# RustAudio/rodio

Measured on AMD Instinct MI355X. Metric: Msamples/s through resample+low_pass+mix pipeline, higher is better.
Workload: dtype f32; 1 GPU; 256 f32 stereo sources/GPU x 1048576 frames, 44.1->48 kHz linear resample + low_pass(200) + ordered Mixer sum, span_len=None; numpy default_rng(1234+s) U(-1,1)/256; in_frames=1048576, out_frames=1141308, channels=2, kernel=k_rlm_chunk

## Files before the change

### rodio_amd/csrc/rh_pipeline_chunk.hip

```cpp
#include "rh_pipeline_dev.h"

namespace {

struct ChunkArgs {
    const uint32_t *m_lo;
    unsigned long long *halo;
    const float *lookT;
    const float *powM;
    const float *uni;
};
constexpr uint32_t kChunkMultiMax = 7;
struct ChunkMulti {
    struct Entry {
        Params p;
        ChunkArgs q;
    };
    uint32_t n;
    uint32_t first[kChunkMultiMax + 1];
    float *sum_out;
    Entry e[kChunkMultiMax];
};
static_assert(sizeof(ChunkMulti) <= 4096, "the kernarg segment");
#if defined(RH_CHUNK_DIAG) && RH_CHUNK_DIAG == 3
#define RH_CPH(i) { const unsigned long long cph_now = __builtin_readcyclecounter(); if (lane == 0) atomicAdd(p.ticket + 8 + (i), (uint32_t)(cph_now - cph_last)); cph_last = cph_now; }
#define RH_CPH_DECL unsigned long long cph_last = __builtin_readcyclecounter();
#else
#define RH_CPH(i)
#define RH_CPH_DECL
#endif
template <int R, int C, int KV, typename ST = float>
__device__ __forceinline__ void rlm_chunk_tile(const Params &p, const ChunkArgs &q, const uint32_t block) {
    typedef Chan<C> CH;
    typedef typename CH::V V;
    constexpr bool PCM = sizeof(ST) == 2;
    constexpr int NS = 2, H = 4;
    constexpr uint32_t FB = CH::kFB;
    constexpr uint32_t kStage = KV * 1024, P = kStage / FB;
    constexpr int NSI = PCM ? 2 * NS : NS;
    constexpr uint32_t kIn = PCM ? kStage / 2 : kStage;
    constexpr int G = PCM ? KV / 2 : KV;
    static_assert(KV % 2 == 0 && NSI * kIn == NS * kStage, "the ring's bytes, cut for either sample type");
    constexpr uint32_t MB = NS * kStage + 64;
    __shared__ __attribute__((aligned(1024))) unsigned char smem[MB + kStage + 64];
    lds_u8 *const lds = (lds_u8 *)smem;
    const uint32_t lds0 = (uint32_t)(uintptr_t)lds;
    typedef __attribute__((address_space(4))) const uint64_t cu64;
    typedef __attribute__((address_space(4))) const float cf32;
    typedef __attribute__((address_space(4))) const uint32_t cu32;
    cu64 *const desc = (cu64 *)(uintptr_t)p.srcs;
    cf32 *const dgain = (cf32 *)(uintptr_t)p.srcs;
    const int lane = threadIdx.x;
    uint32_t tile = block;
    if (!p.direct) {
        const uint32_t x = block & 7u;
        const uint32_t k = __builtin_amdgcn_readfirstlane(lane == 0 ? atomicAdd(p.ticket + 32u * (1u + x), 1u) - p.shard_base : 0u);
        tile = x + 8u * k;
        if (tile >= p.n_tiles) return;
    }
#ifdef RH_CHUNK_RAGSIM
    const uint32_t Ns = p.eq_frames;
    const uint32_t S = 2u * tile < p.n_tiles ? p.n_sources : (uint32_t)(((uint64_t)p.n_sources * 2u * (p.n_tiles - tile)) / p.n_tiles);
#else
    const uint32_t Ns = p.eq_frames, S = p.n_sources;
#endif
    const uint32_t m_lo = ((cu32 *)(uintptr_t)q.m_lo)[tile], m_hi = ((cu32 *)(uintptr_t)q.m_lo)[tile + 1];
    const uint32_t m0 = m_lo + (uint32_t)lane * R;
    int nfl;
    uint32_t n_t_v;
    float pwv[4];
    {
        const uint32_t n_t = m_hi - m_lo;
        nfl = (int)n_t - lane * R < 0 ? 0 : ((int)n_t - lane * R > R ? R : (int)n_t - lane * R);
        const uint32_t nl0 = (n_t + R - 1) / R;
        const uint32_t v = nl0 ? n_t - (nl0 - 1) * R : 0;
        n_t_v = n_t;
        asm volatile("v_mov_b32 %0, %1" : "=v"(n_t_v) : "s"(n_t));
        const float *pw = q.powM + 4 * v;
#pragma unroll
        for (int k = 0; k < 4; ++k) {
            pwv[k] = pw[k];
            asm volatile("" : "+v"(pwv[k]));
        }
    }
    const bool first = (m0 == 0);

    const uint32_t nvec = PCM ? Ns * C / 8 : Ns * C / 4;
    const uint32_t v0 = tile * (G * 64);
    uint32_t goff[G];
#pragma unroll
    for (int k = 0; k < G; ++k) {
        uint32_t j = v0 + (uint32_t)k * 64 + lane;
        j = j < nvec ? j : nvec - 1;
        goff[k] = j * 16;
    }
    const bool lin = v0 + (uint32_t)(G * 64) <= nvec;
    auto stage_source = [&](uint32_t s_, uint32_t stage) {
        const void *data = (const void *)(uintptr_t)desc[4 * (uint64_t)s_];
        if (lin) {
            glds16_run<G>(data, goff[0], lds0 + stage * kIn);
        } else {
#pragma unroll
            for (int k = 0; k < G; ++k) glds16(data, goff[k], lds0 + stage * kIn + k * 1024);
        }
    };
    if (S) stage_source(0, 0);
    if (S > 1) stage_source(1, 1);
    if constexpr (PCM) {
        if (S > 2) stage_source(2, 2);
        if (S > 3) stage_source(3, 3);
    }
    const Tables *__restrict__ tb = p.tabs;
    float lM[4], b15[4], b31[4], kM[4];
    constexpr int NHV = H * FB / 16;
    const uint32_t Jc = p.J < tile ? p.J : tile;
    int want_look = (uint32_t)lane < Jc ? 1 : 0;
    uint64_t a_halo_pub = (uint64_t)(uintptr_t)(q.halo + (uint64_t)tile * 8 + (uint32_t)(lane >= 64 - NHV ? lane - (64 - NHV) : 0) * 4);
    uint64_t a_halo_poll = (uint64_t)(uintptr_t)(q.halo + (uint64_t)(tile ? tile - 1 : 0) * 8 + (lane < H * C ? lane : 0));
    uint64_t a_gran_pub = (uint64_t)(uintptr_t)(p.gran + (uint64_t)tile * 4 + (lane < 2 * C ? lane : 0));
    uint64_t a_gran_poll = (uint64_t)(uintptr_t)(p.gran + (uint64_t)(tile ? tile - 1 - (want_look ? lane : 0) : 0) * 4);
    uint64_t a_out = (uint64_t)(uintptr_t)(p.out + ((uint64_t)m_lo + (uint32_t)lane) * C);
    uint32_t epoch_v = p.epoch;
    float U = q.uni[lane < 61 ? lane : 60];
    asm volatile("" : "+v"(want_look), "+v"(a_halo_pub), "+v"(a_halo_poll), "+v"(a_gran_pub), "+v"(a_gran_poll), "+v"(a_out), "+v"(epoch_v), "+v"(U));
    {
        const uint32_t Jc0 = Jc;
        const float *kp = q.lookT + ((uint64_t)tile * p.J + ((uint32_t)lane < Jc0 ? lane : 0)) * 4;
#pragma unroll
        for (int k = 0; k < 4; ++k) {
            lM[k] = tb->laneM[lane][k];
            b15[k] = tb->bc15M[lane][k];
            b31[k] = tb->bc31M[lane][k];
            kM[k] = kp[k];
        }
    }
    int offA[R + 2];
    float wgt[R + 2];
    {
        const int64_t fbase = (int64_t)tile * P;
        Cursor c = cursor_at(first ? 0 : m0 - 2, p);
#pragma unroll
        for (int rr = 0; rr < R + 2; ++rr) {
#if defined(RH_CHUNK_DIAG) && RH_CHUNK_DIAG == 2
            offA[rr] = (int)MB + rr * 8;
            wgt[rr] = 0.5f;
            continue;
#endif
            const bool dummy = first && rr < 2;
            uint64_t i;
            uint32_t num;
            cursor_resolve(c, p, i, num);
            if (i + 1 >= Ns) {
                i = Ns - 1;
                num = 0;
            }
            int64_t f = (int64_t)i - fbase;
            f = f < -H ? -H : (f > (int64_t)P - 1 ? (int64_t)P - 1 : f);
            offA[rr] = dummy ? (int)MB : (int)MB + (int)f * (int)FB;
            wgt[rr] = dummy ? 0.0f : (float)num / p.Tf;
            if (!dummy) cursor_next(c, p);
        }
    }
    v4f acc[KV];
#pragma unroll
    for (int k = 0; k < KV; ++k) acc[k] = v4f{0.f, 0.f, 0.f, 0.f};
    if constexpr (!PCM) {
        uint32_t st = 0;
        float g_next = S ? dgain[4] : 0.f;
        for (uint32_t s_ = 0; s_ < S; ++s_) {
            const float g = g_next;
            g_next = s_ + 1 < S ? dgain[8 * (uint64_t)(s_ + 1) + 4] : 0.f;
            if (s_ + 1 < S) wait_vm<KV>();
            else wait_vm<0>();
            const lds_u8 *buf = lds + st * kStage;
            v4f v[KV];
#pragma unroll
            for (int k = 0; k < KV; ++k) v[k] = *(const lds_f4 *)(buf + k * 1024 + lane * 16);
            asm volatile("s_waitcnt lgkmcnt(0)" ::: "memory");
            if (s_ + 2 < S) stage_source(s_ + 2, st);
#pragma unroll
            for (int k = 0; k < KV; ++k) {
                acc[k].x = fma_(g, v[k].x, acc[k].x);
                acc[k].y = fma_(g, v[k].y, acc[k].y);
                acc[k].z = fma_(g, v[k].z, acc[k].z);
                acc[k].w = fma_(g, v[k].w, acc[k].w);
            }
            st ^= 1u;
        }
    } else {
        uint32_t st = 0;
        float g_next = S ? dgain[4] : 0.f;
        for (uint32_t s_ = 0; s_ < S; ++s_) {
            const float g = g_next;
            g_next = s_ + 1 < S ? dgain[8 * (uint64_t)(s_ + 1) + 4] : 0.f;
            const uint32_t left = S - 1 - s_;
            wait_groups<G, NSI>((int)(left < (uint32_t)(NSI - 1) ? left : (uint32_t)(NSI - 1)));
            const lds_u8 *buf = lds + st * kIn;
            v4i16 v[KV];
#pragma unroll
            for (int k = 0; k < KV; ++k) v[k] = *(const RH_LDS v4i16 *)(buf + k * 512 + lane * 8);
            asm volatile("s_waitcnt lgkmcnt(0)" ::: "memory");
            if (s_ + NSI < S) stage_source(s_ + NSI, st);
#pragma unroll
            for (int k = 0; k < KV; ++k) {
                acc[k].x = fma_(g, pcm16_f32(v[k].x), acc[k].x);
                acc[k].y = fma_(g, pcm16_f32(v[k].y), acc[k].y);
                acc[k].z = fma_(g, pcm16_f32(v[k].z), acc[k].z);
                acc[k].w = fma_(g, pcm16_f32(v[k].w), acc[k].w);
            }
            st = (st + 1u) & (uint32_t)(NSI - 1);
        }
    }
    RH_CPH_DECL
#if defined(RH_CHUNK_DIAG) && RH_CHUNK_DIAG < 3
    {
        float t = 0.f;
#pragma unroll
        for (int k = 0; k < KV; ++k) t += acc[k].x + acc[k].y + acc[k].z + acc[k].w;
#pragma unroll
        for (int rr = 0; rr < R + 2; ++rr) t += wgt[rr] + (float)offA[rr];
        p.out[(uint64_t)tile * 64 + lane] = t + lM[0] + b15[0] + b31[0] + kM[0] + (float)nfl + (first ? 1.f : 0.f);
        return;
    }
#endif
    if (lane >= 64 - NHV) {
        unsigned long long *hp = (unsigned long long *)(uintptr_t)a_halo_pub;
        const float e[4] = {acc[KV - 1].x, acc[KV - 1].y, acc[KV - 1].z, acc[KV - 1].w};
#pragma unroll
        for (int w = 0; w < 4; ++w) __hip_atomic_store(hp + w, ((unsigned long long)epoch_v << 32) | __float_as_uint(e[w]), __ATOMIC_RELAXED, __HIP_MEMORY_SCOPE_AGENT);
    }
#pragma unroll
    for (int k = 0; k < KV; ++k) *(lds_f4 *)(lds + MB + (uint32_t)(k * 64 + lane) * 16) = acc[k];
    if (lane == 0) *(lds_f4 *)(lds + MB + kStage) = v4f{0.f, 0.f, 0.f, 0.f};
    bool dead = false;
    if (tile == 0) {
        if (lane < H * C) *(RH_LDS float *)(lds + MB - H * FB + lane * 4) = 0.0f;
    } else {
        const bool want = lane < H * C;
        const unsigned long long *hp = (const unsigned long long *)(uintptr_t)a_halo_poll;
        unsigned long long hv = 0;
        bool ok = false;
        uint32_t spins = 0;
        while (true) {
            if (want && !ok) {
                hv = __hip_atomic_load(hp, __ATOMIC_RELAXED, __HIP_MEMORY_SCOPE_AGENT);
                ok = (uint32_t)(hv >> 32) == epoch_v;
            }
            if (__all(ok || !want)) break;
            if (++spins > kSpinLimit) {
                if (lane == 0) atomicOr(p.status, 1u);
                dead = true;
                break;
            }
            __builtin_amdgcn_s_sleep(1);
        }
        if (want) *(RH_LDS float *)(lds + MB - H * FB + lane * 4) = dead ? __builtin_nanf("") : __uint_as_float((uint32_t)hv);
    }
    asm volatile("s_waitcnt lgkmcnt(0)" ::: "memory");
    __builtin_amdgcn_wave_barrier();
    RH_CPH(0)

    const float b0 = readlane_f(U, 0), c1 = readlane_f(U, 1), c2 = readlane_f(U, 2), na1 = -readlane_f(U, 3), na2 = -readlane_f(U, 4);
    V out[R];
    V E1 = CH::zero(), E2 = CH::zero();
    {
        V ta[R + 2], tb2[R + 2];
#pragma unroll
        for (int rr = 0; rr < R + 2; ++rr) {
            ta[rr] = CH::ld_lds(lds + offA[rr]);
            tb2[rr] = CH::ld_lds(lds + offA[rr] + FB);
        }
        auto tap = [&](int rr) -> V {
            V x;
#pragma unroll
            for (int ch = 0; ch < C; ++ch) CH::set(x, ch, fma_(CH::get(tb2[rr], ch) - CH::get(ta[rr], ch), wgt[rr], CH::get(ta[rr], ch)));
            return x;
        };
        V x2 = first ? CH::zero() : tap(0);
        V x1 = first ? CH::zero() : tap(1);
        V w1 = CH::zero(), w2 = CH::zero();
#pragma unroll
        for (int r = 0; r < R; ++r) {
            const V x = tap(r + 2);
            V w;
#pragma unroll
            for (int ch = 0; ch < C; ++ch) {
                const float wc = fma_(na1, CH::get(w1, ch), fma_(na2, CH::get(w2, ch), fma_(c2, CH::get(x2, ch), c1 * CH::get(x1, ch))));
                CH::set(w, ch, wc);
                CH::set(out[r], ch, fma_(b0, CH::get(x, ch), wc));
            }
            w2 = w1;
            w1 = w;
            x2 = x1;
            x1 = x;
            E1 = vsel(r + 1 == nfl, w1, E1);
            E2 = vsel(r + 1 == nfl, w2, E2);
        }
    }
    RH_CPH(1)
    float Pq[2 * C];
#pragma unroll
    for (int k = 0; k < 2 * C; ++k) Pq[k] = 0.f;
    {
        const float Tm[4] = {readlane_f(U, 5), readlane_f(U, 6), readlane_f(U, 7), readlane_f(U, 8)};
#pragma unroll
        for (int ch = 0; ch < C; ++ch) mat_acc(Tm, CH::get(E1, ch), CH::get(E2, ch), Pq[2 * ch], Pq[2 * ch + 1]);
    }
    float own[2 * C];
#pragma unroll
    for (int k = 0; k < 2 * C; ++k) own[k] = Pq[k];
    scan_states(Pq, ScanStepsLanes{U}, b15, b31);
    {
        const uint32_t n_t = (uint32_t)__builtin_amdgcn_readfirstlane((int)n_t_v);
        float A[2 * C];
        tile_aggregate(own, Pq, pwv, (int)((n_t + R - 1) / R), A);
        if (lane < 2 * C) {
            float ev = A[0];
#pragma unroll
            for (int k = 1; k < 2 * C; ++k) ev = lane == k ? A[k] : ev;
            __hip_atomic_store((unsigned long long *)(uintptr_t)a_gran_pub, ((unsigned long long)epoch_v << 32) | __float_as_uint(ev), __ATOMIC_RELAXED, __HIP_MEMORY_SCOPE_AGENT);
        }
    }
    float Q[2 * C];
#pragma unroll
    for (int k = 0; k < 2 * C; ++k) Q[k] = dpp0<kDppWaveShr1, 0xf>(Pq[k]);
    RH_CPH(2)
    float c[2 * C];
#pragma unroll
    for (int k = 0; k < 2 * C; ++k) c[k] = 0.f;
    if (tile > 0) {
        const bool want = want_look != 0;
        const unsigned long long *gp = (const unsigned long long *)(uintptr_t)a_gran_poll;
        unsigned long long gv[2 * C];
#pragma unroll
        for (int k = 0; k < 2 * C; ++k) gv[k] = 0;
        bool ok = false;
        uint32_t spins = 0;
        while (true) {
            if (want && !ok) {
                bool all = true;
#pragma unroll
                for (int k = 0; k < 2 * C; ++k) {
                    gv[k] = __hip_atomic_load(gp + k, __ATOMIC_RELAXED, __HIP_MEMORY_SCOPE_AGENT);
                    all = all && ((uint32_t)(gv[k] >> 32) == epoch_v);
                }
                ok = all;
            }
            if (__all(ok || !want)) break;
            if (++spins > kSpinLimit) {
                if (lane == 0) atomicOr(p.status, 1u);
                dead = true;
                break;
            }
            __builtin_amdgcn_s_sleep(4);
        }
        if (lane == 0 && spins) atomicAdd(p.status + 1, spins);
        if (want && ok && !dead) {
#pragma unroll
            for (int ch = 0; ch < C; ++ch) mat_acc(kM, __uint_as_float((uint32_t)gv[2 * ch]), __uint_as_float((uint32_t)gv[2 * ch + 1]), c[2 * ch], c[2 * ch + 1]);
        }
#pragma unroll
        for (int k = 0; k < 2 * C; ++k) {
            c[k] += dpp0<kDppRowShr + 1, 0xf>(c[k]);
            c[k] += dpp0<kDppRowShr + 2, 0xf>(c[k]);
            c[k] += dpp0<kDppRowShr + 4, 0xf>(c[k]);
            c[k] += dpp0<kDppRowShr + 8, 0xf>(c[k]);
            c[k] = readlane_f(c[k], 15) + readlane_f(c[k], 31);
        }
    }
    if (dead) {
#pragma unroll
        for (int k = 0; k < 2 * C; ++k) c[k] = __builtin_nanf("");
    }
    RH_CPH(3)
#pragma unroll
    for (int ch = 0; ch < C; ++ch) mat_acc(lM, c[2 * ch], c[2 * ch + 1], Q[2 * ch], Q[2 * ch + 1]);
    tile_store<R, C>(lds, lane, [&] { return (uint32_t)__builtin_amdgcn_readfirstlane((int)n_t_v); }, [&] { return (float *)(uintptr_t)a_out; }, [&](int r) {
        V y;
#pragma unroll
        for (int ch = 0; ch < C; ++ch) CH::set(y, ch, fma_(readlane_f(U, 25 + 2 * r), Q[2 * ch], fma_(readlane_f(U, 26 + 2 * r), Q[2 * ch + 1], CH::get(out[r], ch))));
        return y;
    });
    RH_CPH(4)
}
template <int R, int C, int KV>
__global__ __launch_bounds__(64, 2) void k_rlm_chunk(const Params p, const ChunkArgs q) {
    rlm_chunk_tile<R, C, KV>(p, q, blockIdx.x);
}
template <int R, int C, int KV>
__global__ __launch_bounds__(64, 2) void k_rlm_chunk_pcm16(const Params p, const ChunkArgs q) {
    rlm_chunk_tile<R, C, KV, int16_t>(p, q, blockIdx.x);
}
template <int R, int C, int KV>
__global__ __launch_bounds__(64, 2) void k_rlm_chunk_multi(const ChunkMulti m) {
    uint32_t k = 0;
#pragma unroll
    for (uint32_t i = 1; i < kChunkMultiMax; ++i) k += (i < m.n && blockIdx.x >= m.first[i]) ? 1u : 0u;
    uint32_t b0 = 0;
#pragma unroll
    for (uint32_t i = 1; i < kChunkMultiMax; ++i) b0 = (i == k) ? m.first[i] : b0;
    k = __builtin_amdgcn_readfirstlane(k);
    typedef const __attribute__((address_space(4))) unsigned char *cbytes;
    cbytes e = (cbytes)__builtin_amdgcn_kernarg_segment_ptr() + offsetof(ChunkMulti, e) + (size_t)k * sizeof(ChunkMulti::Entry);
    Params p;
    ChunkArgs q;
    typedef const __attribute__((address_space(4))) uint32_t *cwords;
    static_assert(sizeof(Params) % 4 == 0 && sizeof(ChunkArgs) % 4 == 0 && offsetof(ChunkMulti::Entry, q) % 4 == 0, "copied word by word");
    {
        cwords wp = (cwords)(e + offsetof(ChunkMulti::Entry, p)), wq = (cwords)(e + offsetof(ChunkMulti::Entry, q));
        uint32_t *dp = reinterpret_cast<uint32_t *>(&p), *dq = reinterpret_cast<uint32_t *>(&q);
#pragma unroll
        for (uint32_t i = 0; i < sizeof(Params) / 4; ++i) dp[i] = wp[i];
#pragma unroll
        for (uint32_t i = 0; i < sizeof(ChunkArgs) / 4; ++i) dq[i] = wq[i];
    }
    rlm_chunk_tile<R, C, KV>(p, q, blockIdx.x - b0);
}

#if defined(RH_CLS_DIAG) && RH_CLS_DIAG == 9
__device__ unsigned long long g_cls_stamp[2048 * 8 * 8];
#define RH_CLS_STAMP(i) { if (lane == 0 && tile < 2048 && k < 8) g_cls_stamp[((uint64_t)tile * 8 + k) * 8 + (i)] = wall_clock64(); }
#else
#define RH_CLS_STAMP(i)
#endif
#define RH_PARG(T, e, f) (*(const __attribute__((address_space(4))) T *)((e) + offsetof(ChunkMulti::Entry, p) + offsetof(Params, f)))
#define RH_QARG(T, e, f) (*(const __attribute__((address_space(4))) T *)((e) + offsetof(ChunkMulti::Entry, q) + offsetof(ChunkArgs, f)))
template <int R, int C, int KV>
__global__ __launch_bounds__(128, 2) void k_rlm_chunk_classes(const ChunkMulti m) {
    typedef Chan<C> CH;
    typedef typename CH::V V;
    constexpr int NS = 2, H = 4;
    constexpr uint32_t FB = CH::kFB;
    constexpr uint32_t kStage = KV * 1024, P = kStage / FB;
    constexpr uint32_t kCtl = NS * kStage;
    constexpr uint32_t kImg = kStage + 128;
    constexpr uint32_t MB0 = kCtl + 64 + 64;
    __shared__ __attribute__((aligned(1024))) unsigned char smem[kCtl + 64 + 2 * kImg];
    lds_u8 *const lds = (lds_u8 *)smem;
    const uint32_t lds0 = (uint32_t)(uintptr_t)lds;
    typedef __attribute__((address_space(4))) const uint64_t cu64;
    typedef __attribute__((address_space(4))) const float cf32;
    typedef __attribute__((address_space(4))) const uint32_t cu32;
    typedef const __attribute__((address_space(4))) unsigned char *cbytes;
    const cbytes kseg = (cbytes)__builtin_amdgcn_kernarg_segment_ptr();
    const int wave = __builtin_amdgcn_readfirstlane((int)(threadIdx.x >> 6));
    const int lane = (int)(threadIdx.x & 63u);
    const uint32_t n_cls = m.n;
    const Params &p0 = m.e[0].p;
    const uint32_t tile = blockIdx.x;
    const uint32_t Ns = p0.eq_frames;
    auto entry = [&](uint32_t k) -> cbytes { return kseg + offsetof(ChunkMulti, e) + (size_t)k * sizeof(ChunkMulti::Entry); };
    auto ctl_read = [&](uint32_t which) -> uint32_t {
        uint32_t v;
        asm volatile("ds_read_b32 %0, %1\n\ts_waitcnt lgkmcnt(0)" : "=v"(v) : "v"(lds0 + kCtl + which * 4) : "memory");
        return (uint32_t)__builtin_amdgcn_readfirstlane((int)v);
    };
    auto ctl_write = [&](uint32_t which, uint32_t v) {
        asm volatile("s_waitcnt lgkmcnt(0)" ::: "memory");
        if (lane == 0) *(RH_LDS uint32_t *)(lds + kCtl + which * 4) = v;
        asm volatile("s_waitcnt lgkmcnt(0)" ::: "memory");
    };
    if (wave == 0) {
        if (lane < 2) *(RH_LDS uint32_t *)(lds + kCtl + lane * 4) = 0u;
    }
    asm volatile("s_waitcnt lgkmcnt(0)\n\ts_barrier" ::: "memory");
    if (wave == 0) {
        const uint32_t nvec = Ns * C / 4;
        const uint32_t v0 = tile * (KV * 64);
        uint32_t goff[KV];
#pragma unroll
        for (int k = 0; k < KV; ++k) {
            uint32_t j = v0 + (uint32_t)k * 64 + lane;
            j = j < nvec ? j : nvec - 1;
            goff[k] = j * 16;
        }
        const bool lin = v0 + (uint32_t)(KV * 64) <= nvec;
        auto stage_source = [&](cu64 *desc, uint32_t s_, uint32_t stage) {
            const void *data = (const void *)(uintptr_t)desc[4 * (uint64_t)s_];
            if (lin) {
                glds16_run<KV>(data, goff[0], lds0 + stage * kStage);
            } else {
#pragma unroll
                for (int k = 0; k < KV; ++k) glds16(data, goff[k], lds0 + stage * kStage + k * 1024);
            }
        };
        constexpr int NHV = H * FB / 16;
        __builtin_amdgcn_s_setprio(3);
        uint32_t kc = 0, sc = 0;
        cu64 *ndesc = (cu64 *)(uintptr_t)RH_PARG(uint64_t, entry(0), srcs);
        uint32_t nS = RH_PARG(uint32_t, entry(0), n_sources);
        uint32_t nstage = 0;
        auto request_next = [&]() {
            if (kc >= n_cls) return false;
            stage_source(ndesc, sc, nstage);
            nstage ^= 1u;
            if (++sc == nS) {
                sc = 0;
                if (++kc < n_cls) {
                    ndesc = (cu64 *)(uintptr_t)RH_PARG(uint64_t, entry(kc), srcs);
                    nS = RH_PARG(uint32_t, entry(kc), n_sources);
                }
            }
            return true;
        };
        uint32_t ahead = 0;
        if (request_next()) ++ahead;
        if (request_next()) ++ahead;
        uint32_t st = 0;
        for (uint32_t k = 0; k < n_cls; ++k) {
            const cbytes e = entry(k);
            cf32 *const dgain = (cf32 *)(uintptr_t)RH_PARG(uint64_t, e, srcs);
            const uint32_t S = RH_PARG(uint32_t, e, n_sources);
            v4f acc[KV];
#pragma unroll
            for (int i = 0; i < KV; ++i) acc[i] = v4f{0.f, 0.f, 0.f, 0.f};
            float g_next = S ? dgain[4] : 0.f;
            for (uint32_t s_ = 0; s_ < S; ++s_) {
                const float g = g_next;
                g_next = s_ + 1 < S ? dgain[8 * (uint64_t)(s_ + 1) + 4] : 0.f;
                if (ahead > 1) wait_vm<KV>();
                else wait_vm<0>();
                --ahead;
                const lds_u8 *buf = lds + st * kStage;
                v4f v[KV];
#pragma unroll
                for (int i = 0; i < KV; ++i) v[i] = *(const lds_f4 *)(buf + i * 1024 + lane * 16);
                asm volatile("s_waitcnt lgkmcnt(0)" ::: "memory");
                if (request_next()) ++ahead;
#pragma unroll
                for (int i = 0; i < KV; ++i) {
                    acc[i].x = fma_(g, v[i].x, acc[i].x);
                    acc[i].y = fma_(g, v[i].y, acc[i].y);
                    acc[i].z = fma_(g, v[i].z, acc[i].z);
                    acc[i].w = fma_(g, v[i].w, acc[i].w);
                }
                st ^= 1u;
            }
            RH_CLS_STAMP(0)
            if (lane >= 64 - NHV) {
                unsigned long long *hp = (unsigned long long *)(uintptr_t)RH_QARG(uint64_t, e, halo) + (uint64_t)tile * 8 + (uint32_t)(lane - (64 - NHV)) * 4;
                const uint32_t epoch = RH_PARG(uint32_t, e, epoch);
                const float ev[4] = {acc[KV - 1].x, acc[KV - 1].y, acc[KV - 1].z, acc[KV - 1].w};
#pragma unroll
                for (int w = 0; w < 4; ++w) __hip_atomic_store(hp + w, ((unsigned long long)epoch << 32) | __float_as_uint(ev[w]), __ATOMIC_RELAXED, __HIP_MEMORY_SCOPE_AGENT);
            }
            if (k >= 2) {
                uint32_t spins = 0;
                while (ctl_read(1) + 2 <= k) {
                    if (++spins > kSpinLimit) break;
                    __builtin_amdgcn_s_sleep(8);
                }
            }
            {
                lds_u8 *img = lds + MB0 + (k & 1u) * kImg;
#pragma unroll
                for (int i = 0; i < KV; ++i) *(lds_f4 *)(img + (uint32_t)(i * 64 + lane) * 16) = acc[i];
                if (lane == 0) *(lds_f4 *)(img + kStage) = v4f{0.f, 0.f, 0.f, 0.f};
            }
            ctl_write(0, k + 1);
            RH_CLS_STAMP(1)
        }
        return;
    }
    const ChunkArgs &q0 = m.e[0].q;
    const uint32_t m_lo = ((cu32 *)(uintptr_t)q0.m_lo)[tile], m_hi = ((cu32 *)(uintptr_t)q0.m_lo)[tile + 1];
    const uint32_t m0 = m_lo + (uint32_t)lane * R;
    const uint32_t n_t = m_hi - m_lo;
    const int nfl = (int)n_t - lane * R < 0 ? 0 : ((int)n_t - lane * R > R ? R : (int)n_t - lane * R);
    const uint32_t nl0 = (n_t + R - 1) / R;
    const uint32_t vlast = nl0 ? n_t - (nl0 - 1) * R : 0;
    const bool first = (m0 == 0);
    int offA[R + 2];
    float wgt[R + 2];
    {
        const int64_t fbase = (int64_t)tile * P;
        Cursor c = cursor_at(first ? 0 : m0 - 2, p0);
#pragma unroll
        for (int rr = 0; rr < R + 2; ++rr) {
            const bool dummy = first && rr < 2;
            uint64_t i;
            uint32_t num;
            cursor_resolve(c, p0, i, num);
            if (i + 1 >= Ns) {
                i = Ns - 1;
                num = 0;
            }
            int64_t f = (int64_t)i - fbase;
            f = f < -H ? -H : (f > (int64_t)P - 1 ? (int64_t)P - 1 : f);
            offA[rr] = dummy ? 0 : (int)f * (int)FB;
            wgt[rr] = dummy ? 0.0f : (float)num / p0.Tf;
            if (!dummy) cursor_next(c, p0);
        }
    }
    V ytot[R];
#pragma unroll
    for (int r = 0; r < R; ++r) ytot[r] = CH::zero();
    for (uint32_t k = 0; k < n_cls; ++k) {
        const cbytes e = entry(k);
        const Tables *__restrict__ tb = (const Tables *)(uintptr_t)RH_PARG(uint64_t, e, tabs);
        const uint32_t J = RH_PARG(uint32_t, e, J), epoch = RH_PARG(uint32_t, e, epoch);
        const uint32_t Jc = J < tile ? J : tile;
        const bool want_look = (uint32_t)lane < Jc;
        unsigned long long *const halo = (unsigned long long *)(uintptr_t)RH_QARG(uint64_t, e, halo);
        unsigned long long *const gran = (unsigned long long *)(uintptr_t)RH_PARG(uint64_t, e, gran);
        uint32_t *const status = (uint32_t *)(uintptr_t)RH_PARG(uint64_t, e, status);
        const float U = ((const float *)(uintptr_t)RH_QARG(uint64_t, e, uni))[lane < 61 ? lane : 60];
        float lM[4], b15[4], b31[4], kM[4], pwv[4];
        {
            const float *kp = (const float *)(uintptr_t)RH_QARG(uint64_t, e, lookT) + ((uint64_t)tile * J + (want_look ? lane : 0)) * 4;
            const float *pw = (const float *)(uintptr_t)RH_QARG(uint64_t, e, powM) + 4 * vlast;
#pragma unroll
            for (int i = 0; i < 4; ++i) {
                lM[i] = tb->laneM[lane][i];
                b15[i] = tb->bc15M[lane][i];
                b31[i] = tb->bc31M[lane][i];
                kM[i] = kp[i];
                pwv[i] = pw[i];
            }
        }
        lds_u8 *const img = lds + MB0 + (k & 1u) * kImg;
        {
            uint32_t spins = 0;
            while (ctl_read(0) <= k) {
                if (++spins > kSpinLimit) {
                    if (lane == 0) atomicOr(status, 1u);
                    break;
                }
                __builtin_amdgcn_s_sleep(8);
            }
        }
#if defined(RH_CLS_DIAG) && RH_CLS_DIAG == 1
        CH::set(ytot[0], 0, CH::get(ytot[0], 0) + lM[0] + b15[0] + b31[0] + kM[0] + pwv[0] + U + (float)offA[0] + wgt[1] + (float)nfl + (want_look ? 1.f : 0.f) + (float)(uintptr_t)halo + (float)(uintptr_t)gran + (float)(uintptr_t)status + (float)epoch);
        ctl_write(1, k + 1);
        continue;
#endif
        RH_CLS_STAMP(2)
        bool dead = false;
        if (tile == 0) {
            if (lane < H * C) *(RH_LDS float *)(img - H * FB + lane * 4) = 0.0f;
        } else {
            const bool want = lane < H * C;
            const unsigned long long *hp = halo + (uint64_t)(tile - 1) * 8 + (want ? lane : 0);
            unsigned long long hv = 0;
            bool ok = false;
            uint32_t spins = 0;
            while (true) {
                if (want && !ok) {
                    hv = __hip_atomic_load(hp, __ATOMIC_RELAXED, __HIP_MEMORY_SCOPE_AGENT);
                    ok = (uint32_t)(hv >> 32) == epoch;
                }
                if (__all(ok || !want)) break;
                if (++spins > kSpinLimit) {
                    if (lane == 0) atomicOr(status, 1u);
                    dead = true;
                    break;
                }
                __builtin_amdgcn_s_sleep(1);
            }
            if (want) *(RH_LDS float *)(img - H * FB + lane * 4) = dead ? __builtin_nanf("") : __uint_as_float((uint32_t)hv);
        }
        asm volatile("s_waitcnt lgkmcnt(0)" ::: "memory");
        __builtin_amdgcn_wave_barrier();
        RH_CLS_STAMP(3)
        const float b0 = readlane_f(U, 0), c1 = readlane_f(U, 1), c2 = readlane_f(U, 2), na1 = -readlane_f(U, 3), na2 = -readlane_f(U, 4);
        V out[R];
        V E1 = CH::zero(), E2 = CH::zero();
        {
            V ta[R + 2], tb2[R + 2];
#pragma unroll
            for (int rr = 0; rr < R + 2; ++rr) {
                ta[rr] = CH::ld_lds(img + offA[rr]);
                tb2[rr] = CH::ld_lds(img + offA[rr] + FB);
            }
            auto tap = [&](int rr) -> V {
                V x;
#pragma unroll
                for (int ch = 0; ch < C; ++ch) CH::set(x, ch, fma_(CH::get(tb2[rr], ch) - CH::get(ta[rr], ch), wgt[rr], CH::get(ta[rr], ch)));
                return x;
            };
            V x2 = first ? CH::zero() : tap(0);
            V x1 = first ? CH::zero() : tap(1);
            V w1 = CH::zero(), w2 = CH::zero();
#pragma unroll
            for (int r = 0; r < R; ++r) {
                const V x = tap(r + 2);
                V w;
#pragma unroll
                for (int ch = 0; ch < C; ++ch) {
                    const float wc = fma_(na1, CH::get(w1, ch), fma_(na2, CH::get(w2, ch), fma_(c2, CH::get(x2, ch), c1 * CH::get(x1, ch))));
                    CH::set(w, ch, wc);
                    CH::set(out[r], ch, fma_(b0, CH::get(x, ch), wc));
                }
                w2 = w1;
                w1 = w;
                x2 = x1;
                x1 = x;
                E1 = vsel(r + 1 == nfl, w1, E1);
                E2 = vsel(r + 1 == nfl, w2, E2);
            }
        }
        float Pq[2 * C];
#pragma unroll
        for (int i = 0; i < 2 * C; ++i) Pq[i] = 0.f;
        {
            const float Tm[4] = {readlane_f(U, 5), readlane_f(U, 6), readlane_f(U, 7), readlane_f(U, 8)};
#pragma unroll
            for (int ch = 0; ch < C; ++ch) mat_acc(Tm, CH::get(E1, ch), CH::get(E2, ch), Pq[2 * ch], Pq[2 * ch + 1]);
        }
        float own[2 * C];
#pragma unroll
        for (int i = 0; i < 2 * C; ++i) own[i] = Pq[i];
#define RH_CSCAN(K, N)                                                                             \
    {                                                                                              \
        float sq[2 * C];                                                                           \
        _Pragma("unroll") for (int i = 0; i < 2 * C; ++i) sq[i] = dpp0<kDppRowShr + N, 0xf>(Pq[i]); \
        const float sM[4] = {readlane_f(U, 9 + 4 * K), readlane_f(U, 10 + 4 * K), readlane_f(U, 11 + 4 * K), readlane_f(U, 12 + 4 * K)}; \
        _Pragma("unroll") for (int ch = 0; ch < C; ++ch) mat_acc(sM, sq[2 * ch], sq[2 * ch + 1], Pq[2 * ch], Pq[2 * ch + 1]); \
    }
        RH_CSCAN(0, 1)
        RH_CSCAN(1, 2)
        RH_CSCAN(2, 4)
        RH_CSCAN(3, 8)
#undef RH_CSCAN
        {
            float sq[2 * C];
#pragma unroll
            for (int i = 0; i < 2 * C; ++i) sq[i] = dpp0<kDppBcast15, 0xa>(Pq[i]);
#pragma unroll
            for (int ch = 0; ch < C; ++ch) mat_acc(b15, sq[2 * ch], sq[2 * ch + 1], Pq[2 * ch], Pq[2 * ch + 1]);
        }
        {
            float sq[2 * C];
#pragma unroll
            for (int i = 0; i < 2 * C; ++i) sq[i] = dpp0<kDppBcast31, 0xc>(Pq[i]);
#pragma unroll
            for (int ch = 0; ch < C; ++ch) mat_acc(b31, sq[2 * ch], sq[2 * ch + 1], Pq[2 * ch], Pq[2 * ch + 1]);
        }
        {
            const int nl = (int)nl0;
            float A[2 * C];
#pragma unroll
            for (int i = 0; i < 2 * C; ++i) A[i] = 0.f;
            if (nl >= 1) {
#pragma unroll
                for (int i = 0; i < 2 * C; ++i) A[i] = __int_as_float(__builtin_amdgcn_readlane(__float_as_int(own[i]), nl - 1));
            }
            if (nl >= 2) {
                const float M[4] = {readfirstlane_f(pwv[0]), readfirstlane_f(pwv[1]), readfirstlane_f(pwv[2]), readfirstlane_f(pwv[3])};
                float xp[2 * C];
#pragma unroll
                for (int i = 0; i < 2 * C; ++i) xp[i] = __int_as_float(__builtin_amdgcn_readlane(__float_as_int(Pq[i]), nl - 2));
#pragma unroll
                for (int ch = 0; ch < C; ++ch) mat_acc(M, xp[2 * ch], xp[2 * ch + 1], A[2 * ch], A[2 * ch + 1]);
            }
            if (lane < 2 * C) {
                float ev = A[0];
#pragma unroll
                for (int i = 1; i < 2 * C; ++i) ev = lane == i ? A[i] : ev;
                __hip_atomic_store(gran + (uint64_t)tile * 4 + (uint32_t)lane, ((unsigned long long)epoch << 32) | __float_as_uint(ev), __ATOMIC_RELAXED, __HIP_MEMORY_SCOPE_AGENT);
            }
        }
        float Q[2 * C];
#pragma unroll
        for (int i = 0; i < 2 * C; ++i) Q[i] = dpp0<kDppWaveShr1, 0xf>(Pq[i]);
        float c[2 * C];
#pragma unroll
        for (int i = 0; i < 2 * C; ++i) c[i] = 0.f;
        if (tile > 0) {
            const unsigned long long *gp = gran + (uint64_t)(tile - 1 - (want_look ? (uint32_t)lane : 0u)) * 4;
            unsigned long long gv[2 * C];
#pragma unroll
            for (int i = 0; i < 2 * C; ++i) gv[i] = 0;
            bool ok = false;
            uint32_t spins = 0;
            while (true) {
                if (want_look && !ok) {
                    bool all = true;
#pragma unroll
                    for (int i = 0; i < 2 * C; ++i) {
                        gv[i] = __hip_atomic_load(gp + i, __ATOMIC_RELAXED, __HIP_MEMORY_SCOPE_AGENT);
                        all = all && ((uint32_t)(gv[i] >> 32) == epoch);
                    }
                    ok = all;
                }
                if (__all(ok || !want_look)) break;
                if (++spins > kSpinLimit) {
                    if (lane == 0) atomicOr(status, 1u);
                    dead = true;
                    break;
                }
                __builtin_amdgcn_s_sleep(4);
            }
            if (lane == 0 && spins) atomicAdd(status + 1, spins);
            if (want_look && ok && !dead) {
#pragma unroll
                for (int ch = 0; ch < C; ++ch) mat_acc(kM, __uint_as_float((uint32_t)gv[2 * ch]), __uint_as_float((uint32_t)gv[2 * ch + 1]), c[2 * ch], c[2 * ch + 1]);
            }
            half_wave_sum(c);
        }
        if (dead) {
#pragma unroll
            for (int i = 0; i < 2 * C; ++i) c[i] = __builtin_nanf("");
        }
#pragma unroll
        for (int ch = 0; ch < C; ++ch) mat_acc(lM, c[2 * ch], c[2 * ch + 1], Q[2 * ch], Q[2 * ch + 1]);
        RH_CLS_STAMP(4)
        ctl_write(1, k + 1);
#pragma unroll
        for (int r = 0; r < R; ++r) {
#pragma unroll
            for (int ch = 0; ch < C; ++ch) {
                const float y = fma_(readlane_f(U, 25 + 2 * r), Q[2 * ch], fma_(readlane_f(U, 26 + 2 * r), Q[2 * ch + 1], CH::get(out[r], ch)));
                CH::set(ytot[r], ch, CH::get(ytot[r], ch) + y);
            }
        }
        RH_CLS_STAMP(5)
    }
    {
        constexpr uint32_t kRow = (R + 1) * FB;
        static_assert(64 * kRow <= kCtl + 64 + 2 * kImg, "the rows fit the LDS (the ring, and behind it the images: everything is free now)");
        lds_u8 *row = lds + (uint32_t)lane * kRow;
#pragma unroll
        for (int r = 0; r < R; ++r) {
            if (C == 2) *(lds_f2 *)(row + r * FB) = v2f{CH::get(ytot[r], 0), CH::get(ytot[r], C - 1)};
            else *(RH_LDS float *)(row + r * FB) = CH::get(ytot[r], 0);
        }
        asm volatile("s_waitcnt lgkmcnt(0)" ::: "memory");
        __builtin_amdgcn_wave_barrier();
        float *ot = m.sum_out + ((uint64_t)m_lo + (uint32_t)lane) * C;
        for (uint32_t f0 = 0; f0 < n_t; f0 += 64) {
            const uint32_t f = f0 + (uint32_t)lane;
            if (f < n_t) {
                const lds_u8 *src2 = lds + (f / R) * kRow + (f % R) * FB;
                if (C == 2) {
                    const v2f a = *(const lds_f2 *)src2;
                    *reinterpret_cast<float2 *>(ot + (uint64_t)f0 * 2) = make_float2(a.x, a.y);
                } else {
                    ot[f0] = *(const RH_LDS float *)src2;
                }
            }
        }
    }
}
#undef RH_PARG
#undef RH_QARG

}

namespace rhp {

struct ChunkInst {
    uint32_t C;
    int R, KV;
    const void *one, *multi, *classes;
    const void *pcm16 = nullptr;
};
#define RH_FN(k) reinterpret_cast<const void *>(&k)
static const ChunkInst kChunk[] = {
    {2, 9, 4, RH_FN((k_rlm_chunk<9, 2, 4>)), RH_FN((k_rlm_chunk_multi<9, 2, 4>)), nullptr},
    {2, 18, 8, RH_FN((k_rlm_chunk<18, 2, 8>)), RH_FN((k_rlm_chunk_multi<18, 2, 8>)), RH_FN((k_rlm_chunk_classes<18, 2, 8>)), RH_FN((k_rlm_chunk_pcm16<18, 2, 8>))},
    {2, 18, 4, RH_FN((k_rlm_chunk<18, 2, 4>)), RH_FN((k_rlm_chunk_multi<18, 2, 4>)), RH_FN((k_rlm_chunk_classes<18, 2, 4>)), RH_FN((k_rlm_chunk_pcm16<18, 2, 4>))},
    {1, 18, 4, RH_FN((k_rlm_chunk<18, 1, 4>)), RH_FN((k_rlm_chunk_multi<18, 1, 4>)), RH_FN((k_rlm_chunk_classes<18, 1, 4>)), RH_FN((k_rlm_chunk_pcm16<18, 1, 4>))},
    {1, 18, 2, RH_FN((k_rlm_chunk<18, 1, 2>)), RH_FN((k_rlm_chunk_multi<18, 1, 2>)), RH_FN((k_rlm_chunk_classes<18, 1, 2>)), RH_FN((k_rlm_chunk_pcm16<18, 1, 2>))},
};
#undef RH_FN
static const ChunkInst *chunk_inst(int R, uint32_t channels, int KV) {
    for (const ChunkInst &c : kChunk)
        if (c.C == channels && c.R == R && c.KV == KV) return &c;
    return nullptr;
}
const void *chunk_kernel(int R, uint32_t channels, int KV) {
    const ChunkInst *c = chunk_inst(R, channels, KV);
    return c ? c->one : nullptr;
}
const void *chunk_kernel_pcm16(int R, uint32_t channels, int KV) {
    const ChunkInst *c = chunk_inst(R, channels, KV);
    return c ? c->pcm16 : nullptr;
}

static void chunk_params(const rh_rlm *p, Params &k, ChunkArgs &ca) {
    const ChunkPlan &c = p->chunk;
    k.tabs = c.d_tabs;
    k.gran = c.d_gran;
    k.n_tiles = c.n_tiles;
    k.J = c.J;
    k.u = c.uni;
    ca.m_lo = c.d_mlo;
    ca.halo = c.d_halo;
    ca.lookT = c.d_look;
    ca.powM = c.d_pow;
    ca.uni = c.d_uni;
    k.direct = (c.direct && p->exclusive) ? 1u : 0u;
}

rh_status chunk_launch_classes(rh_rlm *const *classes, float *const *rows, uint64_t row_capacity_frames, uint32_t n, float *dst_sum, rh_stream stream, bool *taken, bool *summed) {
    *taken = false;
    *summed = false;
    if (n < 2 || n > kChunkMultiMax || rh::knob(rh::K_CLASSES_ONE_BY_ONE)) return RH_OK;
    const ChunkInst *inst = nullptr;
    for (uint32_t k = 0; k < n; ++k) {
        const rh_rlm *h = classes[k];
        if (!h || !h->cls.empty() || !h->plan || h->out_frames == 0 || row_capacity_frames < h->out_frames) return RH_OK;
        if (rh::rlm::route(route_in(h, *h->plan)) != rh::rlm::kChunk) return RH_OK;
        const ChunkInst *c = chunk_inst(h->chunk.R, h->cfg.channels, h->chunk.KV);
        if (!c || !c->multi || (inst && c->multi != inst->multi)) return RH_OK;
        inst = c;
    }
    RH_REQUIRE_INIT();
    for (uint32_t k = 0; k < n; ++k)
        if (!rows[k] || (reinterpret_cast<uintptr_t>(rows[k]) & 15u)) return RH_ERR_INVALID;
    hipStream_t s = rh::as_stream(stream);
    ChunkMulti m;
    memset(&m, 0, sizeof m);
    for (uint32_t k = 0; k < n; ++k) {
        rh_rlm *h = classes[k];
        rh_status w = pre_launch(h, s);
        if (w == RH_OK) w = next_epoch(h, s);
        if (w != RH_OK) return w;
        m.e[k].p = launch_params(h, *h->plan, 0, h->n_sources, rows[k], 0, 0, StreamArgs{});
        chunk_params(h, m.e[k].p, m.e[k].q);
        m.e[k].p.direct = 0;
        m.first[k + 1] = m.first[k] + rh::rlm::sharded_grid(h->chunk.n_tiles);
    }
    m.n = n;
    void *args[] = {&m};
    const void *fn2 = rh::knob(rh::K_CLASSES_ONE_WAVE) ? nullptr : inst->classes;
    bool same = fn2 != nullptr;
    for (uint32_t k = 0; k < n && same; ++k) {
        const rh_rlm *h = classes[k], *h0 = classes[0];
        same = h->exclusive && h->eq_frames == h0->eq_frames && h->out_frames == h0->out_frames && h->F == h0->F && h->T == h0->T && h->chunk_in == h0->chunk_in &&
               h->chunk_out == h0->chunk_out && h->chunk.n_tiles == h0->chunk.n_tiles && h->chunk.R == h0->chunk.R && h->chunk.KV == h0->chunk.KV && h->n_sources >= 1;
    }
    if (same) {
        int per_cu = 0;
        same = hipOccupancyMaxActiveBlocksPerMultiprocessor(&per_cu, fn2, 128, 0) == hipSuccess && per_cu >= 1 &&
               (uint64_t)classes[0]->chunk.n_tiles <= (uint64_t)per_cu * (uint64_t)rh::g_num_cus;
    }
    if (same) m.sum_out = dst_sum;
    const hipError_t e = same ? hipLaunchKernel(fn2, dim3(classes[0]->chunk.n_tiles), dim3(128), args, 0, s) : hipLaunchKernel(inst->multi, dim3(m.first[n]), dim3(64), args, 0, s);
    if (e != hipSuccess) {
        rh::set_hip_error(e, "k_rlm_chunk_multi / k_rlm_chunk_classes launch");
        return RH_ERR_HIP;
    }
    *summed = same;
    for (uint32_t k = 0; k < n; ++k) {
        rh::rlm::booked(&classes[k]->tk, same, rh::rlm::kShards, m.first[k + 1] - m.first[k]);
        mark_launch(classes[k], s);
    }
    *taken = true;
    return RH_OK;
}

#if defined(RH_CLS_DIAG) && RH_CLS_DIAG == 9
extern "C" int rh_debug_cls_stamps(unsigned long long *dst, size_t n) {
    return (int)hipMemcpyFromSymbol(dst, HIP_SYMBOL(g_cls_stamp), n * sizeof(unsigned long long), 0, hipMemcpyDeviceToHost);
}
#endif

rh_status launch_chunk(rh_rlm *p, Params &k, hipStream_t s, bool pcm16) {
    ChunkArgs ca;
    chunk_params(p, k, ca);
    if (pcm16) {
        k.srcs = p->d_pcm;
        k.direct = (p->chunk.direct_pcm && p->exclusive) ? 1u : 0u;
    }
    const uint32_t grid = k.direct ? k.n_tiles : rh::rlm::sharded_grid(k.n_tiles);
    void *args[] = {&k, &ca};
    const hipError_t e = hipLaunchKernel(pcm16 ? p->chunk.fn_pcm : p->chunk.fn, dim3(grid), dim3(64), args, 0, s);
    if (e != hipSuccess) {
        rh::set_hip_error(e, "k_rlm_chunk launch");
        return RH_ERR_HIP;
    }
    rh::rlm::booked(&p->tk, k.direct != 0, rh::rlm::kShards, grid);
    return mark_launch(p, s);
}

}
```

Measured before the change: 1.682 million Msamples/s.

## Interleave resample tap computation into the f32 source-mix loop via LDS table

For the f32 chunk kernel, the per-row resample tap offsets and weights are no longer computed in a dedicated loop before the mix. One tap row is computed per source iteration inside the source-summing loop, written to an LDS table, and read back into registers after the loop. The aim is to hide the cursor arithmetic under the memory waits of the staged source loads and to cut register pressure from carrying offA/wgt live across the loop. The cost is extra shared memory, extra LDS traffic, and a fallback loop when there are fewer sources than tap rows.

Result: no change. 1.698 million Msamples/s (median of 6 runs) (+1.0%).

```diff
diff --git a/rodio_amd/csrc/rh_pipeline_chunk.hip b/rodio_amd/csrc/rh_pipeline_chunk.hip
--- a/rodio_amd/csrc/rh_pipeline_chunk.hip
+++ b/rodio_amd/csrc/rh_pipeline_chunk.hip
@@ -28,11 +28,12 @@
 #define RH_CPH(i)
 #define RH_CPH_DECL
 #endif
-template <int R, int C, int KV, typename ST = float>
+template <int R, int C, int KV, typename ST = float, bool TUL = false>
 __device__ __forceinline__ void rlm_chunk_tile(const Params &p, const ChunkArgs &q, const uint32_t block) {
     typedef Chan<C> CH;
     typedef typename CH::V V;
     constexpr bool PCM = sizeof(ST) == 2;
+    static_assert(!PCM || !TUL, "the 16-bit source loop keeps its form");
     constexpr int NS = 2, H = 4;
     constexpr uint32_t FB = CH::kFB;
     constexpr uint32_t kStage = KV * 1024, P = kStage / FB;
@@ -41,7 +42,9 @@
     constexpr int G = PCM ? KV / 2 : KV;
     static_assert(KV % 2 == 0 && NSI * kIn == NS * kStage, "the ring's bytes, cut for either sample type");
     constexpr uint32_t MB = NS * kStage + 64;
-    __shared__ __attribute__((aligned(1024))) unsigned char smem[MB + kStage + 64];
+    constexpr uint32_t kTab = NS * kStage, kTabBytes = TUL ? (R + 2) * 64 * 8 : 0;
+    constexpr uint32_t kSmem = MB + kStage + 64 > kTab + kTabBytes ? MB + kStage + 64 : kTab + kTabBytes;
+    __shared__ __attribute__((aligned(1024))) unsigned char smem[kSmem];
     lds_u8 *const lds = (lds_u8 *)smem;
     const uint32_t lds0 = (uint32_t)(uintptr_t)lds;
     typedef __attribute__((address_space(4))) const uint64_t cu64;
@@ -135,7 +138,29 @@
     }
     int offA[R + 2];
     float wgt[R + 2];
-    {
+    Cursor tc;
+    auto tap_step = [&](const uint32_t rr) {
+#if defined(RH_CHUNK_DIAG) && RH_CHUNK_DIAG == 2
+        *(lds_f2 *)(lds + kTab + (rr * 64u + (uint32_t)lane) * 8u) = v2f{__int_as_float((int)MB + (int)rr * 8), 0.5f};
+        return;
+#endif
+        if (rr == 0) tc = cursor_at(first ? 0 : m0 - 2, p);
+        const bool dummy = first && rr < 2;
+        uint64_t i;
+        uint32_t num;
+        cursor_resolve(tc, p, i, num);
+        if (i + 1 >= Ns) {
+            i = Ns - 1;
+            num = 0;
+        }
+        int64_t f = (int64_t)i - (int64_t)tile * P;
+        f = f < -H ? -H : (f > (int64_t)P - 1 ? (int64_t)P - 1 : f);
+        const int off = dummy ? (int)MB : (int)MB + (int)f * (int)FB;
+        const float w = dummy ? 0.0f : (float)num / p.Tf;
+        *(lds_f2 *)(lds + kTab + (rr * 64u + (uint32_t)lane) * 8u) = v2f{__int_as_float(off), w};
+        if (!dummy) cursor_next(tc, p);
+    };
+    if constexpr (!TUL) {
         const int64_t fbase = (int64_t)tile * P;
         Cursor c = cursor_at(first ? 0 : m0 - 2, p);
 #pragma unroll
@@ -185,6 +210,18 @@
                 acc[k].w = fma_(g, v[k].w, acc[k].w);
             }
             st ^= 1u;
+            if constexpr (TUL) {
+                if (s_ < (uint32_t)(R + 2)) tap_step(s_);
+            }
+        }
+        if constexpr (TUL) {
+            for (uint32_t rr = S; rr < (uint32_t)(R + 2); ++rr) tap_step(rr);
+#pragma unroll
+            for (int rr = 0; rr < R + 2; ++rr) {
+                const v2f e = *(const lds_f2 *)(lds + kTab + ((uint32_t)rr * 64u + (uint32_t)lane) * 8u);
+                offA[rr] = __float_as_int(e.x);
+                wgt[rr] = e.y;
+            }
         }
     } else {
         uint32_t st = 0;
@@ -384,7 +421,7 @@
 }
 template <int R, int C, int KV>
 __global__ __launch_bounds__(64, 2) void k_rlm_chunk(const Params p, const ChunkArgs q) {
-    rlm_chunk_tile<R, C, KV>(p, q, blockIdx.x);
+    rlm_chunk_tile<R, C, KV, float, true>(p, q, blockIdx.x);
 }
 template <int R, int C, int KV>
 __global__ __launch_bounds__(64, 2) void k_rlm_chunk_pcm16(const Params p, const ChunkArgs q) {
```
